# randomwons/RayTracingStudy

Measured on AMD Instinct MI355X. Metric: Mrays/s (primary+shadow) at 1920x1080, 64 spp, 100000 spheres, higher is better.
Workload: dtype f32; 1 GPU; c3: 64 spp Monte-Carlo accumulate, ~100k spheres (headline); width=1920, height=1080, spp=64, n_spheres=100000, octree_depth=7, octree_nodes=37384, prim_refs=153448, leaf_capacity=12, parallelism=single, frames_in_flight=1, rays_per_frame=184963628, primary_per_frame=132710400

## Files before the change

### include/rt.h

```cpp
#ifndef RT_AMD_RT_H
#define RT_AMD_RT_H

#include <stddef.h>
#include <stdint.h>

#ifdef __cplusplus
extern "C" {
#endif

#define RT_ABI_VERSION 4

typedef struct rt_renderer rt_renderer;

enum {
    RT_OK = 0,
    RT_E_INVALID = -1,
    RT_E_HIP = -2,
    RT_E_NOMEM = -3,
    RT_E_NOSCENE = -4,
    RT_E_STATE = -5
};

enum {
    RT_MODE_COMPAT = 0,
    RT_MODE_SCENE = 1
};

enum {
    RT_FLAG_JITTER = 1u << 0,
    RT_FLAG_NO_JITTER = 1u << 1,
    RT_FLAG_RADIANCE = 1u << 2,
    RT_FLAG_NO_SHADOWS = 1u << 3,
    RT_FLAG_HOST_BUILD = 1u << 4,
    RT_FLAG_PROGRESSIVE = 1u << 5,
    RT_FLAG_COMPAT_FMA = 1u << 6,
    RT_FLAG_PAD_FILL_SHIFT = 8,
    RT_FLAG_TEST_HOOKS = 1u << 10,
    RT_FLAG_TEST_POISON = 1u << 11,
    RT_FLAG_NO_OCCLUDERS = 1u << 12,
    RT_FLAG_NO_BINS = 1u << 13,
    RT_FLAG_VARIANT_SHIFT = 16,
    RT_FLAG_OPT_SHIFT = 20,
    RT_FLAG_CELL_TABLE_SHIFT = 28
};

typedef struct rt_config {
    uint32_t width;
    uint32_t height;
    uint32_t spp;
    uint32_t seed;
    int32_t device;
    uint32_t mode;
    uint32_t flags;
    float light_dir[3];
    float ambient;
} rt_config;

typedef struct rt_octree_params {
    float min[3];
    float max[3];
    float resolution;
    uint32_t max_depth;
    uint32_t leaf_capacity;
// ... 58 lines not shown
    RT_BINS_ON = 0,
    RT_BINS_OFF_FLAG = 1,
    RT_BINS_OFF_KERNEL = 2,
    RT_BINS_OFF_CAMERA = 3,
    RT_BINS_OFF_CAPACITY = 4,
    RT_BINS_OFF_WIDE = 5,
    RT_BINS_OFF_DENSE = 6,
    RT_BINS_NO_FRAME = 7
};
typedef struct rt_bin_info {
    uint32_t enabled;
    uint32_t reason;
    uint32_t bin_size;
    uint32_t bins;
    uint32_t entries;
    uint32_t capacity;
    uint32_t non_empty_bins;
    uint32_t longest;
    uint32_t overflowed_bins;
    uint32_t wide;
    float bin_build_ms;
} rt_bin_info;
int rt_get_bin_info(rt_renderer* r, rt_bin_info* info);
int rt_export_bins(rt_renderer* r, uint32_t* headers_out, uint32_t* indices_out, uint32_t* wide_out);
int rt_export_bin_tiles(rt_renderer* r, uint32_t* tw, uint32_t* th, uint32_t* tiles_per_bin,
                        uint64_t* words_out);
int rt_generate_spheres(uint32_t n, uint32_t seed, float* spheres_out, uint32_t* albedo_out);

int rt_save_spheres(const char* path, const float* spheres, const uint32_t* albedo, uint32_t n);
int rt_load_spheres(const char* path, float* spheres_out, uint32_t* albedo_out,
                    uint32_t capacity, uint32_t* n_out);

int rt_render(rt_renderer* r, void* dev_rgba8, void* stream, rt_stats* stats);
int rt_bind_graphics_resource(rt_renderer* r, void* hip_graphics_resource);
typedef struct rt_display_ops {
    int (*map)(void* user, void* stream, void** dev_ptr, size_t* bytes);
    int (*unmap)(void* user, void* stream);
} rt_display_ops;
int rt_bind_display(rt_renderer* r, const rt_display_ops* ops, void* user);
int rt_render_tiles(rt_renderer* r, const uint32_t* tile_ids, uint32_t n_tiles,
                    uint32_t tile_size, void* dev_packed_rgba8, void* stream, rt_stats* stats);
#define RT_TILE_SKIP 0xFFFFFFFFu
int rt_unpack_tiles(rt_renderer* r, const void* dev_packed_rgba8, const uint32_t* tile_ids,
                    uint32_t n_tiles, uint32_t tile_size, void* dev_rgba8, void* stream);
int rt_reset_accumulation(rt_renderer* r);
int rt_synchronize(rt_renderer* r);
// ... 99 lines not shown
```

### raytracingstudy_amd/_lib.py

```python
from __future__ import annotations

import ctypes
import os
import threading

_HERE = os.path.dirname(os.path.abspath(__file__))
LIB_PATH = os.environ.get("RT_AMD_LIB") or os.path.join(_HERE, "librt_amd.so")

RT_OK = 0
RT_E_INVALID = -1
RT_E_HIP = -2
RT_E_NOMEM = -3
RT_E_NOSCENE = -4
RT_E_STATE = -5

RT_MODE_COMPAT = 0
RT_MODE_SCENE = 1

RT_FLAG_JITTER = 1 << 0
RT_FLAG_NO_JITTER = 1 << 1
RT_FLAG_RADIANCE = 1 << 2
RT_FLAG_NO_SHADOWS = 1 << 3
RT_FLAG_HOST_BUILD = 1 << 4
RT_FLAG_PROGRESSIVE = 1 << 5
RT_FLAG_COMPAT_FMA = 1 << 6
RT_BUILDER_DEVICE = 0
RT_BUILDER_HOST = 1
RT_TILE_SKIP = 0xFFFFFFFF
RT_FLAG_PAD_FILL_SHIFT = 8
RT_FLAG_TEST_HOOKS = 1 << 10
RT_FLAG_TEST_POISON = 1 << 11
RT_FLAG_NO_OCCLUDERS = 1 << 12
RT_FLAG_NO_BINS = 1 << 13
RT_FLAG_VARIANT_SHIFT = 16
RT_FLAG_OPT_SHIFT = 20
RT_FLAG_CELL_TABLE_SHIFT = 28
RT_CELL_TABLE_OFF = 15
VARIANT_REMOVED = 2
VARIANT_BLOCK = 7
VARIANT_WAVEQ = 13
VARIANT_WAVEQ_LOW = 4
RT_TRANSPORT_AUTO = 0
RT_TRANSPORT_RCCL = 1
RT_TRANSPORT_PEER = 2
RT_MAX_DEVICES = 16
RT_NO_HIT = 0xFFFFFFFF
RT_QUERY_NEAREST = 0
RT_QUERY_ANY = 1
RT_MULTIHIT_MAX = 16
RT_OVERLAP_MAX = 16
RT_OVERLAP_MORE = 0x80000000
RT_OVERLAP_SKIP_SELF = 1
RT_CLOSEST_MAX = 16
RT_CLOSEST_SKIP_SELF = 1
RT_SWEEP_ENTRY_ONLY = 1
RT_SWEEP_SKIP_SELF = 2
# ... 159 lines not shown
_P = ctypes.c_void_p
_u32 = ctypes.c_uint32
_int = ctypes.c_int
_fp = ctypes.POINTER(ctypes.c_float)
SIGNATURES = {
    "rt_abi_version": (_int, []),
    "rt_device_count": (_int, []),
    "rt_config_default": (None, [ctypes.POINTER(RtConfig)]),
    "rt_octree_params_default": (None, [ctypes.POINTER(RtOctreeParams)]),
    "rt_create": (_int, [ctypes.POINTER(RtConfig), ctypes.POINTER(_P)]),
    "rt_destroy": (_int, [_P]),
    "rt_set_pose": (_int, [_P, _fp]),
    "rt_set_intrinsic": (_int, [_P, _fp]),
    "rt_get_camera": (_int, [_P, _fp, _fp]),
    "rt_resize": (_int, [_P, _u32, _u32]),
    "rt_resize_intrinsic": (None, [_u32, _u32, _fp]),
    "rt_set_scene": (_int, [_P, _P, _P, _u32, ctypes.POINTER(RtOctreeParams)]),
    "rt_set_scene_device": (_int, [_P, _P, _P, _u32, ctypes.POINTER(RtOctreeParams), _P]),
    "rt_set_octree": (_int, [_P, _fp, _fp, ctypes.c_float]),
    "rt_get_scene_info": (_int, [_P, ctypes.POINTER(RtSceneInfo)]),
    "rt_export_octree": (_int, [_P, _P, _P, _P]),
    "rt_export_occluders": (_int, [_P, _P, _P, _P, _P]),
    "rt_get_bin_info": (_int, [_P, ctypes.POINTER(RtBinInfo)]),
    "rt_export_bins": (_int, [_P, _P, _P, _P]),
    "rt_export_bin_tiles": (_int, [_P, _P, _P, _P, _P]),
    "rt_save_spheres": (_int, [ctypes.c_char_p, _P, _P, _u32]),
    "rt_load_spheres": (_int, [ctypes.c_char_p, _P, _P, _u32, ctypes.POINTER(_u32)]),
    "rt_generate_spheres": (_int, [_u32, _u32, _P, _P]),
    "rt_render": (_int, [_P, _P, _P, ctypes.POINTER(RtStats)]),
    "rt_bind_graphics_resource": (_int, [_P, _P]),
    "rt_bind_display": (_int, [_P, ctypes.POINTER(RtDisplayOps), _P]),
    "rt_render_tiles": (_int, [_P, _P, _u32, _u32, _P, _P, ctypes.POINTER(RtStats)]),
    "rt_unpack_tiles": (_int, [_P, _P, _P, _u32, _u32, _P, _P]),
    "rt_trace_rays": (_int, [_P, _P, _u32, _u32, _P, _P, ctypes.POINTER(RtStats)]),
    "rt_pick": (_int, [_P, ctypes.c_float, ctypes.c_float, ctypes.POINTER(RtHit), _fp]),
    "rt_trace_rays_multi": (_int, [_P, _P, _u32, _u32, _P, _P, _P, ctypes.POINTER(RtStats)]),
    "rt_pick_multi": (_int, [_P, ctypes.c_float, ctypes.c_float, _u32, ctypes.POINTER(RtHit),
                             ctypes.POINTER(_u32)]),
    "rt_query_overlaps": (_int, [_P, _P, _u32, _u32, _u32, _P, _P, _P, ctypes.POINTER(RtStats)]),
    "rt_overlaps_at": (_int, [_P, _fp, ctypes.c_float, _u32, ctypes.POINTER(_u32), ctypes.POINTER(_u32)]),
    "rt_query_closest": (_int, [_P, _P, _u32, _u32, _u32, _P, _P, _P, ctypes.POINTER(RtStats)]),
    "rt_closest_at": (_int, [_P, _fp, ctypes.c_float, _u32, ctypes.POINTER(RtNear), ctypes.POINTER(_u32)]),
    "rt_sweep_spheres": (_int, [_P, _P, _P, ctypes.c_float, _u32, _u32, _P, _P, ctypes.POINTER(RtStats)]),
    "rt_sweep_at": (_int, [_P, _fp, _fp, ctypes.c_float, ctypes.c_float, _u32, ctypes.POINTER(RtHit), _fp]),
    "rt_pick_thick": (_int, [_P, ctypes.c_float, ctypes.c_float, ctypes.c_float, ctypes.POINTER(RtHit), _fp]),
    "rt_render_gbuffer": (_int, [_P, ctypes.POINTER(RtGBuffer), _P, ctypes.POINTER(RtStats)]),
# ... 70 lines not shown
```

### raytracingstudy_amd/csrc/rt_capi.cpp

```cpp
#include <mutex>

#include "rt_host.h"

using namespace rtamd;

namespace rtamd {

thread_local std::string g_last_error;

int fail(rt_renderer* r, int code, const std::string& msg) {
    g_last_error = msg;
    if (r) r->err = msg;
    return code;
}

int hip_fail(rt_renderer* r, hipError_t e, const char* what) {
    std::string m = std::string(what) + ": " + hipGetErrorString(e);
    return fail(r, RT_E_HIP, m);
}

int set_device(rt_renderer* r) {
    RT_HIP(r, hipSetDevice(r->device));
    return RT_OK;
}
// ... 362 lines not shown
    if ((st = set_device(r))) return st;
    RT_HIP(r, hipStreamSynchronize(r->stream));
    if (r->pending) RT_HIP(r, hipEventSynchronize(r->done));
    occ_collect_time(r);
    return queue_report(r);
}

int rt_readback(rt_renderer* r, uint8_t* host_rgba8, float* host_rgba32f) {
    if (const int st = rt_synchronize(r)) return st;
    const size_t px = (size_t)r->W * r->H;
    if (host_rgba8) RT_HIP(r, hipMemcpy(host_rgba8, r->fb.p, px * 4, hipMemcpyDeviceToHost));
    if (host_rgba32f) {
        if (!(r->cfg.flags & RT_FLAG_RADIANCE))
            return fail(r, RT_E_STATE, "rt_readback: radiance buffer needs RT_FLAG_RADIANCE");
        RT_HIP(r, hipMemcpy(host_rgba32f, r->rad.p, px * 16, hipMemcpyDeviceToHost));
    }
    return RT_OK;
}

void* rt_framebuffer(rt_renderer* r) { return r ? r->fb.p : nullptr; }

void* rt_stream(rt_renderer* r) { return r ? static_cast<void*>(own_stream(r)) : nullptr; }

const char* rt_last_error(const rt_renderer* r) {
    if (r) return r->err.c_str();
    return g_last_error.c_str();
}

}
```

### raytracingstudy_amd/csrc/rt_frame.cpp

```cpp
#include "rt_frame_math.h"
#include "rt_host.h"

using namespace rtamd;

namespace rtamd {

void fill_frame_args(rt_renderer* r, FrameArgs& a) {
    memset(&a, 0, sizeof(a));
    fill_camera(r, a.cam);
    a.sc = r->sc;
    a.W = r->W;
    a.H = r->H;
    a.spp = r->cfg.spp ? r->cfg.spp : 1;
    a.seedmix = mix32(r->cfg.seed ^ 0x9E3779B9u);
    bool jitter = a.spp > 1;
    if (r->cfg.flags & RT_FLAG_JITTER) jitter = true;
    if (r->cfg.flags & RT_FLAG_NO_JITTER) jitter = false;
    a.jitter = jitter ? 1u : 0u;
    a.shadows = (r->cfg.flags & RT_FLAG_NO_SHADOWS) ? 0u : 1u;
    a.contract = (r->cfg.flags & RT_FLAG_COMPAT_FMA) ? 1u : 0u;
    const float* ld = r->cfg.light_dir;
    const float ll = sqrtf(ld[0] * ld[0] + ld[1] * ld[1] + ld[2] * ld[2]);
    a.L[0] = -(ld[0] / ll);
    a.L[1] = -(ld[1] / ll);
    a.L[2] = -(ld[2] / ll);
    a.ambient = r->cfg.ambient;
    a.inv_spp = 1.0f / static_cast<float>(a.spp);
    if ((r->cfg.flags & RT_FLAG_PROGRESSIVE) && r->cfg.mode == RT_MODE_SCENE) {
        if (uint64_t(r->frames_accum + 1) * a.spp >= (1ull << 31)) r->frames_accum = 0;
        a.accum = r->accum.p;
        a.s_base = r->frames_accum * a.spp;
        a.accum_in = r->frames_accum ? 1u : 0u;
        a.inv_spp = 1.0f / static_cast<float>((r->frames_accum + 1) * a.spp);
    }
    a.counters = r->counters.p;
    a.sc.opt = (r->cfg.flags >> RT_FLAG_OPT_SHIFT) & 0xFFu;
    a.wq_claim_delay = r->test_claim_delay;
    a.qerr = r->qerr_dev;
    if (++r->frame_seq == 0) r->frame_seq = 1;
    a.frame_id = r->frame_seq;
    const uint32_t v = (r->cfg.flags >> RT_FLAG_VARIANT_SHIFT) & 0xFu;
    a.variant = v ? v : default_variant(a.spp);
}

int check_tiles(rt_renderer* r, const uint32_t* ids, uint32_t n_tiles, uint32_t ts,
                bool allow_skip) {
    if (ts == 0 || ts % 64 != 0 || ts > 4096)
        return fail(r, RT_E_INVALID, "tile_size must be a multiple of 64 in [64, 4096]");
    const uint32_t tx = (r->W + ts - 1) / ts, ty = (r->H + ts - 1) / ts;
    for (uint32_t i = 0; i < n_tiles; ++i)
        if (ids[i] >= tx * ty && !(allow_skip && ids[i] == RT_TILE_SKIP))
            return fail(r, RT_E_INVALID, "tile id out of range");
    return RT_OK;
}

constexpr size_t kTileListSlots = 16;

int tile_list(rt_renderer* r, const uint32_t* ids, uint32_t n, hipStream_t s, const uint32_t** out) {
    rt_renderer::TileList* hit = nullptr;
// ... 232 lines not shown
    return RT_OK;
}
int block_stats_end(rt_renderer* r, const FrameArgs& a, hipStream_t st) {
    if (!a.bstats) return RT_OK;
    unsigned long long h[2 * kBlockStats];
    RT_HIP(r, hipStreamSynchronize(st));
    RT_HIP(r, hipMemcpy(h, g_bstats, sizeof(h), hipMemcpyDeviceToHost));
    if (FILE* f = fopen(getenv("RT_BLOCK_STATS_FILE"), "a")) {
        fprintf(f, "{\"W\": %u, \"H\": %u, \"spp\": %u, \"counts\": [", a.W, a.H, a.spp);
        for (uint32_t i = 0; i < 2 * kBlockStats; ++i) fprintf(f, "%s%llu", i ? ", " : "", h[i]);
        fprintf(f, "]}\n");
        fclose(f);
    }
    return RT_OK;
}
#else
inline int block_stats_begin(rt_renderer*, FrameArgs&, hipStream_t) { return RT_OK; }
inline int block_stats_end(rt_renderer*, const FrameArgs&, hipStream_t) { return RT_OK; }
#endif

int launch_frame(rt_renderer* r, FrameArgs& a, const FramePlan* plan, hipStream_t st) {
    int ost;
    if ((ost = timeline_begin(r, a, st)) || (ost = block_stats_begin(r, a, st))) return ost;
    hipError_t e = plan ? launch_scene(a, *plan, st) : launch_compat(a, st);
    counters_after_launch(r, a, e == hipSuccess);
    if (e != hipSuccess) return hip_fail(r, e, "kernel launch");
    if ((ost = block_stats_end(r, a, st)) || (ost = mark_queued(r, st))) return ost;
    if ((ost = timeline_end(r, a, st))) return ost;
    if (a.accum) ++r->frames_accum;
    return RT_OK;
}

int frame_stats(rt_renderer* r, const FrameArgs& a, hipStream_t st, rt_stats* stats) {
    RT_HIP(r, hipEventRecord(r->ev1, st));
    RT_HIP(r, hipEventSynchronize(r->ev1));
    occ_collect_time(r);
    unsigned long long lines[kStatLineWords], c[4];
    RT_HIP(r, hipMemcpy(lines, a.counters + kStatLineBase, sizeof(lines), hipMemcpyDeviceToHost));
    sum_stat_lines(lines, c);
    float ms = 0.f;
    RT_HIP(r, hipEventElapsedTime(&ms, r->ev0, r->ev1));
    memset(stats, 0, sizeof(*stats));
    const uint64_t px = a.tiles ? 0 : (uint64_t)a.W * a.H;
    stats->primary_rays = r->cfg.mode == RT_MODE_SCENE ? c[0] : px;
    stats->shadow_rays = c[1];
    stats->nodes_visited = c[2];
    stats->prims_tested = c[3];
// ... 118 lines not shown
```

### raytracingstudy_amd/csrc/rt_host.h

```cpp
#pragma once
#include <hip/hip_runtime.h>
#include <math.h>
#include <stdio.h>
#include <string.h>

#include <algorithm>
#include <chrono>
#include <string>
#include <vector>

#include "../../include/rt.h"
#include "octree_gpu.h"
#include "rt_bins_math.h"
#include "rt_closest_math.h"
#include "rt_overlap_math.h"
#include "rt_params.h"
#include "rt_sweep_math.h"
#include "scene_build.h"

struct ncclComm;

namespace rtamd {

hipError_t launch_scene(const FrameArgs& a, const FramePlan& plan, hipStream_t st);
bool variant_available(uint32_t v);
hipError_t launch_compat(const FrameArgs& a, hipStream_t st);
hipError_t launch_unpack(const uint32_t* packed, const uint32_t* tiles, uint32_t n_tiles,
                         uint32_t ts, uint32_t tiles_x, uint32_t W, uint32_t H, uint32_t* img,
                         hipStream_t st);
hipError_t launch_cam_screen(const float4* prim_sp, uint32_t n, const float o[3], float4* out,
                             hipStream_t st);
hipError_t launch_shd_screen(const float4* prim_sp, uint32_t n, const float e[6], double delta,
                             float2* out8, uint32_t* rr_max, hipStream_t st);
hipError_t launch_albedo_refs(const uint32_t* prim_idx, const uint32_t* albedo, uint32_t n,
                              uint32_t n_spheres, uint32_t* out, hipStream_t st);
hipError_t launch_cam8_screen(const float4* prim_sp, uint32_t n, const float o[3], const float B[9],
                              uint32_t ok, float2* out, hipStream_t st);
hipError_t launch_query(const FrameArgs& a, const void* rays, void* hits, uint32_t n, bool any,
                        unsigned long long* counters, hipStream_t st);
hipError_t launch_multihit(const FrameArgs& a, const void* rays, void* hits, void* counts, uint32_t n,
                           uint32_t k, unsigned long long* counters, hipStream_t st);
hipError_t launch_overlap(const FrameArgs& a, const void* probes, void* indices, void* counts,
                          uint32_t n, uint32_t k, bool skip_self, float slack_m,
                          unsigned long long* counters, hipStream_t st);
hipError_t launch_closest(const FrameArgs& a, const void* probes, void* near, void* counts, uint32_t n,
                          uint32_t k, bool skip_self, float slack_m, unsigned long long* counters,
                          hipStream_t st);
// ... 203 lines not shown
    uint64_t accum_sig = 0;
    DevBuf<unsigned long long> counters;
    size_t ctr_stride = 0;
    uint32_t ctr_set = 0;
    size_t ctr_zero[2] = {0, 0};
    DevBuf<uint32_t> sb_order;
    uint32_t sb_nx = 0, sb_ny = 0;
    struct TileList {
        std::vector<uint32_t> host;
        DevBuf<uint32_t> dev;
        uint64_t used = 0;
    };
    std::vector<TileList> tile_lists;
    uint64_t tile_clock = 0;
    rt_display_ops disp{};
    void* disp_user = nullptr;
    bool gl_disp = false;
    uint32_t n_spheres = 0;
    std::vector<float> spheres;
    bool host_copy = false;
    uint32_t prim_slots = 0;
    bool leaf_packed = false;
    uint32_t test_claim_delay = 0;
    bool sort_rounds = true, lds_stage = true, leaf_pack = false, sb_hilbert = false;
    rt_octree_params oct;
    bool has_scene = false;
    GpuOctreeBuilder gpu_build;
    CellTable cell_table;
    DevBuf<uint2> d_nodes;
    DevBuf<float4> d_prim_sp;
    DevBuf<uint32_t> d_prim_idx;
    DevBuf<float4> d_spheres;
    DevBuf<uint32_t> d_albedo;
    SceneArgs sc{};
    uint64_t scene_gen = 0;
    DerivedRecords<float4> prim_cam;
    DerivedRecords<float2> prim_cam8;
    DerivedRecords<float2> prim_shd8;
    DevBuf<uint32_t> d_shd_rr;
    uint32_t shd_rr_bits = 0;
    float shd_rr = 0.0f;
    DerivedRecords<uint32_t> prim_al;
    OccluderLists occ;
    uint32_t occ_cap = kOccCap;
    double occ_mean_max = kOccMeanMax;
    hipEvent_t occ_e0 = nullptr, occ_e1 = nullptr;
// ... 68 lines not shown
```

### raytracingstudy_amd/csrc/rt_kernels.hip

```cpp
#include <hip/hip_runtime.h>

#include <algorithm>
#include <mutex>
#include <vector>

#include "rt_params.h"
#include "rt_shade.h"
#include "rt_sorted.h"

namespace rtamd {

__device__ __forceinline__ unsigned long long wave_sum(unsigned long long v) {
#pragma unroll
    for (int off = 32; off > 0; off >>= 1) v += __shfl_xor(v, off, 64);
    return v;
}

__device__ __forceinline__ void flush_counters(const FrameArgs& a, uint32_t prim, uint32_t shadow,
                                               uint32_t nodes, uint32_t prims) {
    const unsigned long long s0 = prim;
    const unsigned long long s1 = shadow;
    const unsigned long long s2 = wave_sum(nodes);
    const unsigned long long s3 = wave_sum(prims);
    if ((threadIdx.x & 63u) == 0) {
// ... 118 lines not shown
                    const uint32_t vc = min(8u, nbx - sx * 8u);
                    const uint32_t r2 = r1 - sx * vr * 8u;
                    sx0 = (sx * 8u + r2 % vc) * 8u;
                    sy0 = (sy * 8u + r2 / vc) * 8u;
                }
                if (kTiles) {
                    const uint32_t tile = a.tiles[k];
                    const uint32_t ts = a.tile_size;
                    tox = (tile % a.tiles_x) * ts;
                    toy = (tile / a.tiles_x) * ts;
                    obase = k * ts * ts - toy * ts - tox;
                }
            }
            for (uint32_t cur = w0; cur < w0 + chunk; ++cur) {
                const uint32_t b = cur >> 6, w = cur & 63u;
                const uint32_t wx = sx0 + (b & 7u) * 8u + (w & 7u);
                const uint32_t wy = sy0 + (b >> 3) * 8u + (w >> 3);
                if (wx >= gw || wy >= gh) continue;
                const uint32_t olx = wx * tw, oly = wy * th;
                const uint32_t ox = olx + tox, oy = oly + toy;
#ifdef RT_TIMELINE
                const unsigned long long tu0 = wall_clock64();
#endif
                if (kSort)
                    shade_pixel_sorted<C>(a, wl, stk, ox, oy, obase, n_primary, n_shadow, n_nodes,
                                          n_prims, bs);
                else
                    shade_wave_tile<C>(a, acc, stk, ox, oy, obase, n_primary, n_shadow, n_nodes,
                                       n_prims, bs, lbs, binc);
#ifdef RT_TIMELINE
                const uint32_t sbt = k * sb_grid + (wy >> 6) * nsx + (wx >> 6);
                const unsigned long long uid = (unsigned long long)sbt * 4096u +
                                               (((wy >> 3) & 7u) * 8u + ((wx >> 3) & 7u)) * 64u +
                                               (wy & 7u) * 8u + (wx & 7u);
                if (a.timeline && (threadIdx.x & 63u) == 0 && uid < (1ull << 22)) {
                    const unsigned hw = __builtin_amdgcn_s_getreg((31 << 11) | 4);
                    const unsigned xcc = __builtin_amdgcn_s_getreg((3 << 11) | 20);
                    a.timeline[4ull * 65536 + 3 * uid] = tu0;
                    a.timeline[4ull * 65536 + 3 * uid + 1] = wall_clock64();
                    a.timeline[4ull * 65536 + 3 * uid + 2] =
                        ((unsigned long long)hw << 32) | (xcc << 16) | (blockIdx.x * 4u + wave);
                }
#endif
            }
        }
    } else {
// ... 129 lines not shown
    const size_t lds = C::waveq ? p.lds_bytes : block_tile_lds(p.lds_bytes, p.spw, a.sc.opt);
    const Occupancy o = occupancy(reinterpret_cast<const void*>(kernel), lds);
    uint32_t grid;
    if constexpr (C::waveq) {
        const WaveQueueLaunch s =
            size_wave_queue(p.grid.units(), o.resident, o.cus, C::min_waves, p.ticket, p.ticket_forced);
        a.wq_chunk = s.ticket;
        grid = s.grid;
    } else {
        const BlockTileLaunch s =
            size_block_tiles(a.W, a.H, a.tiles ? a.n_tiles : 0u, a.tile_size, p.grid.tw, p.grid.th,
                             o.resident, (a.sc.opt >> kOptBtsShift) & 7u);
        a.bts = s.side;
        grid = s.grid;
    }
    hipLaunchKernelGGL(kernel, dim3(grid), dim3(kBlockThreads), lds, st, a);
}

template <uint32_t kT>
static bool launch_flags(uint32_t flags, const FrameArgs& a, const FramePlan& p, hipStream_t st) {
    switch (flags) {
#define RT_INSTANCE(f) \
    case (f): launch_instance<Frame<(f) | kT>>(a, p, st); return true;
#define RT_INSTANCE_OCC(f) RT_INSTANCE(f) RT_INSTANCE((f) | kFOcc)
#define RT_INSTANCE_OCC_BIN(f) RT_INSTANCE_OCC(f) RT_INSTANCE_OCC((f) | kFBin)
        RT_INSTANCE(kFStats)
        RT_INSTANCE(kFStats | kFProg)
        RT_INSTANCE(kFStats | kFWaveQ)
        RT_INSTANCE(kFStats | kFWaveQ | kFProg)
        RT_INSTANCE(kFStats | kFWaveQ | kFSorted)
        RT_INSTANCE(kFStats | kFWaveQ | kFSorted | kFProg)
        RT_INSTANCE_OCC(0u)
        RT_INSTANCE_OCC(kFProg)
        RT_INSTANCE_OCC_BIN(kFWaveQ)
        RT_INSTANCE_OCC_BIN(kFWaveQ | kFProg)
        RT_INSTANCE_OCC_BIN(kFWaveQ | kFSorted)
        RT_INSTANCE_OCC_BIN(kFWaveQ | kFSorted | kFProg)
#undef RT_INSTANCE_OCC_BIN
#undef RT_INSTANCE_OCC
#undef RT_INSTANCE
    }
    return false;
}

bool variant_available(uint32_t v) {
    return pick_scene_instance(v, 1, false, false, false, false, false, 0, 1).valid;
}

hipError_t launch_scene(const FrameArgs& a_in, const FramePlan& p, hipStream_t st) {
    FrameArgs a = a_in;
    const SceneInstance inst =
        p.inst.with(a.sc.prim_occ && a.sc.occ_sp && a.shadows, a.bin_hdr && a.bin_ent && a.bin_info);
    a.spw = p.spw, a.g = p.g, a.ppw = p.ppw, a.rounds = p.rounds;
    a.tw = p.grid.tw, a.th = p.grid.th;
    a.wq_chunk = p.ticket;
    const bool known = inst.valid && (a.tiles ? launch_flags<kFTiles>(inst.flags(), a, p, st)
                                              : launch_flags<0u>(inst.flags(), a, p, st));
    return known ? hipGetLastError() : hipErrorInvalidDeviceFunction;
}

}
```

### raytracingstudy_amd/csrc/rt_sched.h

```cpp
#pragma once
#include <stddef.h>
#include <stdint.h>

#ifdef __HIPCC__
#define RT_HD __host__ __device__
#else
#define RT_HD
#endif

namespace rtamd {

constexpr int kBlockThreads = 256;
constexpr uint32_t kTileSide = 16;

constexpr uint32_t kOptBtsShift = 1;
constexpr uint32_t kOptNoWgCap = 1u << 7;
constexpr uint32_t kOptChunkShift = 4;
constexpr uint32_t kOptChunkMax = 4;

constexpr uint32_t kVariantLaneUnified = 7;
constexpr uint32_t kVariantLaneUnified2NoStats = 10;
constexpr uint32_t kVariantWaveQ = 13;
constexpr uint32_t kVariantWaveQLow = 4;
RT_HD inline uint32_t default_variant(uint32_t spp) { return spp >= 8u ? kVariantWaveQ : kVariantWaveQLow; }

constexpr uint32_t kLeafBuf = 32;
constexpr size_t kLeafBufBytes = (kBlockThreads / 64u) * kLeafBuf * 16u;

constexpr uint32_t kSortMaxRounds = 4;
constexpr uint32_t kSortMax = 64u * kSortMaxRounds;
constexpr uint32_t kSortCellBits = 3;
constexpr uint32_t kSortCells = 1u << (2u * kSortCellBits);
constexpr uint32_t kSortWaveBytes = kSortMax * 8u + 3u * kSortMax + kSortCells * 4u;
static_assert(kSortWaveBytes % 16u == 0u, "per-wave regions stay float4-aligned");

RT_HD inline uint32_t stack_levels(uint32_t tab_k, uint32_t stack_depth, bool no_stack = false) {
    if (no_stack && tab_k) return 0u;
    const uint32_t sb = tab_k ? tab_k - 1u : 0u;
    return stack_depth > 1u + sb ? stack_depth - 1u - sb : 1u;
}

// ... 34 lines not shown
        wave_tile_shape(spp, spw, g, ppw, tw, th);
        gw = n_tiles ? tile_size / tw : (W + tw - 1) / tw;
        gh = n_tiles ? tile_size / th : (H + th - 1) / th;
        nbx = (gw + 7u) / 8u, nby = (gh + 7u) / 8u;
        nsx = (nbx + 7u) / 8u, nsy = (nby + 7u) / 8u;
        grids = n_tiles ? n_tiles : 1u;
    }
    RT_HD uint64_t units() const { return static_cast<uint64_t>(grids) * gw * gh; }
    RT_HD uint32_t blocks() const { return grids * nbx * nby; }
    RT_HD uint32_t superblocks() const { return grids * nsx * nsy; }
    RT_HD uint32_t slot_shift() const { return wave_queue_slot_shift(superblocks(), blocks()); }
    RT_HD uint32_t slot_stride() const { return (slot_shift() == 12u ? superblocks() : blocks()) + 2u; }
};


enum FrameFlag : uint32_t {
    kFTiles = 1u << 0,
    kFStats = 1u << 1,
    kFProg = 1u << 2,
    kFWaveQ = 1u << 3,
    kFSorted = 1u << 4,
    kFOcc = 1u << 5,
    kFBin = 1u << 6,
};

template <uint32_t kF>
struct Frame {
    static constexpr bool tiles = kF & kFTiles, stats = kF & kFStats, prog = kF & kFProg,
                          waveq = kF & kFWaveQ, sorted = kF & kFSorted, occ = kF & kFOcc,
                          bin = kF & kFBin;
    static constexpr int min_waves = waveq ? (stats ? 7 : 8) : 1;
    static constexpr bool cam8 = waveq && !sorted;
    static_assert(!sorted || waveq, "sorted rounds: a wave-queue frame");
    static_assert(!occ || !stats, "stats frames walk: their counters are the oracle's");
    static_assert(!bin || (!stats && waveq), "bins: plain frames of the wave queue");
};

struct SceneInstance {
    bool valid;
    bool waveq, stats, prog, sorted, occ, bin;
    RT_HD uint32_t flags() const {
        return (stats ? kFStats : 0u) | (prog ? kFProg : 0u) | (waveq ? kFWaveQ : 0u) |
               (sorted ? kFSorted : 0u) | (occ ? kFOcc : 0u) | (bin ? kFBin : 0u);
    }
    RT_HD uint32_t min_waves() const { return waveq ? (stats ? 7u : 8u) : 1u; }
    RT_HD bool w8() const { return waveq && !stats; }
    RT_HD SceneInstance with(bool have_occ, bool have_bins) const {
        SceneInstance s = *this;
        s.occ = !stats && have_occ;
        s.bin = !stats && waveq && have_bins;
        return s;
    }
};

RT_HD inline SceneInstance pick_scene_instance(uint32_t variant, uint32_t spp, bool progressive,
                                               bool count_work, bool sort_on, bool have_occ,
                                               bool have_bins, uint32_t tab_k, uint32_t stack_depth) {
    if (!variant) variant = default_variant(spp);
    SceneInstance s = {true, false, count_work, progressive, false, false, false};
    const uint32_t rounds = (spp + 63u) / 64u;
    s.sorted = sort_on && spp >= 64u && rounds >= 2u && rounds <= kSortMaxRounds &&
               FrameLds(true, tab_k, stack_depth).bytes * 8u <= 160u * 1024u &&
               (progressive || variant == kVariantWaveQ);
    if (s.sorted)
        s.waveq = true;
    else if (progressive)
        s.waveq = spp >= 8u;
    else if (variant == kVariantWaveQ || variant == kVariantWaveQLow)
        s.waveq = true;
    else if (variant == kVariantLaneUnified)
        s.stats = true;
    else if (variant != kVariantLaneUnified2NoStats)
        s.valid = false;
    return s.with(have_occ, have_bins);
}


struct FramePlan {
    SceneInstance inst;
    WaveGrid grid;
    uint32_t spw, g, ppw, rounds;
    uint32_t slot_shift, slot_stride;
    uint32_t lds_bytes;
    uint32_t ticket;
    bool ticket_forced;
};

RT_HD inline FramePlan plan_scene_frame(uint32_t variant, uint32_t spp, bool progressive, bool count_work,
                                        bool sort_on, uint32_t tab_k, uint32_t stack_depth, uint32_t W,
                                        uint32_t H, uint32_t n_tiles, uint32_t tile_size, uint32_t opt) {
    FramePlan p = {pick_scene_instance(variant, spp, progressive, count_work, sort_on, false, false, tab_k,
                                       stack_depth),
                   WaveGrid(W, H, spp, n_tiles, tile_size)};
    uint32_t tw, th;
    wave_tile_shape(spp, p.spw, p.g, p.ppw, tw, th);
    p.rounds = (spp + p.spw - 1) / p.spw;
    p.slot_shift = p.grid.slot_shift();
    p.slot_stride = p.grid.slot_stride();
    p.lds_bytes = FrameLds(p.inst.sorted, tab_k, stack_depth).bytes;
    const uint32_t ck = (opt >> kOptChunkShift) & 7u;
    p.ticket = ck ? 1u << (ck - 1u) : 4u / (p.rounds < 1u ? 1u : p.rounds > 4u ? 4u : p.rounds);
    p.ticket_forced = ck != 0u;
    return p;
}


struct WaveQueueLaunch {
    uint32_t grid, ticket;
};
struct BlockTileLaunch {
    uint32_t grid, side;
};

RT_HD inline WaveQueueLaunch size_wave_queue(uint64_t units, uint32_t resident, uint32_t cus, uint32_t per_simd,
                                        uint32_t ticket, bool ticket_forced) {
    const uint64_t want = (units + kBlockThreads / 64 - 1) / (kBlockThreads / 64);
    const uint64_t cap = per_simd ? static_cast<uint64_t>(cus) * per_simd : resident;
    uint64_t grid = resident < cap ? resident : cap;
    if (want < grid) grid = want;
    if (grid < 1u) grid = 1u;
    WaveQueueLaunch s = {static_cast<uint32_t>(grid), ticket};
    if (!ticket_forced) {
        const uint64_t per_wave = units / (grid * (kBlockThreads / 64));
        const uint32_t most = per_wave >= 64 ? 4u : per_wave >= 16 ? 2u : 1u;
        if (most < s.ticket) s.ticket = most;
    }
// ... 29 lines not shown
```

### raytracingstudy_amd/csrc/rt_shade.h

```cpp
#pragma once
#include <hip/hip_runtime.h>

#include "rt_params.h"
#include "rt_walk.h"
#include "rt_bins.h"

namespace rtamd {

__device__ __forceinline__ float sat(float x) { return x > 0.0f ? (x < 1.0f ? x : 1.0f) : 0.0f; }

__device__ __forceinline__ uint32_t mix32(uint32_t x) {
    x ^= x >> 16;
    x *= 0x7feb352du;
    x ^= x >> 15;
    x *= 0x846ca68bu;
    x ^= x >> 16;
    return x;
}

__device__ __forceinline__ float u01(uint32_t x) {
    return static_cast<float>(x >> 8) * (1.0f / 16777216.0f);
}

__device__ __forceinline__ void get_ray(const CamArgs& c, float u, float v, float& wx, float& wy,
// ... 165 lines not shown
                c.b = A.z + c.b;
            }
            acc[threadIdx.x] = make_float4(c.r, c.g, c.b, 0.0f);
        }
    }
    KernArgs* ko = kernargs();
    if (leader) {
        const float4 A = acc[threadIdx.x];
        if (kProg) ko->accum[(size_t)y * ko->W + x] = A;
        const float isp = ko->inv_spp;
        const PixelOut p{A.x * isp, A.y * isp, A.z * isp};
        const uint32_t rgba = pack_rgba8(p);
        if (kTiles) {
            ko->out8[obase + y * ko->tile_size + x] = rgba;
        } else {
            ko->out8[(size_t)y * ko->W + x] = rgba;
            if (ko->out32) ko->out32[(size_t)y * ko->W + x] = make_float4(p.r, p.g, p.b, 1.0f);
        }
    } else if (kTiles && sub == 0 && pix < ko->ppw) {
        ko->out8[obase + y * ko->tile_size + x] = 0u;
    }
}

}
```

### raytracingstudy_amd/renderer.py

```python
from __future__ import annotations

import ctypes
from typing import Optional, Sequence

import numpy as np

from . import _lib
from ._lib import (RT_FLAG_HOST_BUILD, RT_FLAG_JITTER, RT_FLAG_NO_JITTER, RT_FLAG_NO_SHADOWS,
                   RT_FLAG_PROGRESSIVE, RT_FLAG_RADIANCE,
                   RT_MODE_COMPAT, RT_MODE_SCENE, RtConfig, RtOctreeParams, RtSceneInfo,
                   RtStats, check)

__all__ = ["KernelRenderer", "resize_intrinsic", "generate_spheres", "device_count",
           "save_spheres", "load_spheres"]

_MODES = {"compat": RT_MODE_COMPAT, "scene": RT_MODE_SCENE}
_QUERY_KINDS = {"nearest": _lib.RT_QUERY_NEAREST, "any": _lib.RT_QUERY_ANY}


def _fptr(a: np.ndarray):
    return a.ctypes.data_as(ctypes.POINTER(ctypes.c_float))


def _vptr(a: Optional[np.ndarray]):
# ... 62 lines not shown
    return sp[:n.value], al[:n.value]


def _octree_params(root_min, root_max, resolution, max_depth, leaf_capacity) -> RtOctreeParams:
    p = RtOctreeParams()
    for i in range(3):
        p.min[i] = float(root_min[i])
        p.max[i] = float(root_max[i])
    p.resolution = float(resolution)
    p.max_depth = int(max_depth)
    p.leaf_capacity = int(leaf_capacity)
    return p


class KernelRenderer:

    def __init__(self, width: int, height: int, *, mode: str = "compat", spp: int = 1,
                 seed: int = 0x2545F491, device: int = -1, jitter: Optional[bool] = None,
                 shadows: bool = True, radiance: bool = False,
                 light_dir: Sequence[float] = (1.0, 1.0, -1.0), ambient: float = 0.1,
                 variant: int = 0, opt_off: int = 0, host_build: bool = False,
                 progressive: bool = False, cell_table: Optional[int] = None,
                 compat_fma: bool = False, pad_fill: int = 0, occluders: bool = True,
                 bins: bool = True,
                 devices: Optional[Sequence[int]] = None, transport: str = "auto"):
        lib = _lib.load()
        cfg = RtConfig()
        lib.rt_config_default(ctypes.byref(cfg))
        cfg.width, cfg.height = int(width), int(height)
        cfg.spp = int(spp)
        cfg.seed = int(seed) & 0xFFFFFFFF
        cfg.device = int(device)
        cfg.mode = _MODES[mode]
        flags = 0
        if jitter is True:
            flags |= RT_FLAG_JITTER
        elif jitter is False:
            flags |= RT_FLAG_NO_JITTER
        if not shadows:
            flags |= RT_FLAG_NO_SHADOWS
        if radiance:
            flags |= RT_FLAG_RADIANCE
        if host_build:
            flags |= RT_FLAG_HOST_BUILD
        if progressive:
            flags |= RT_FLAG_PROGRESSIVE
        if compat_fma:
            flags |= _lib.RT_FLAG_COMPAT_FMA
        if not occluders:
            flags |= _lib.RT_FLAG_NO_OCCLUDERS
        if not bins:
            flags |= _lib.RT_FLAG_NO_BINS
        if not 0 <= int(pad_fill) <= 2:
            raise ValueError("pad_fill must be 0, 1 or 2")
        flags |= int(pad_fill) << _lib.RT_FLAG_PAD_FILL_SHIFT
        flags |= (int(variant) & 0xF) << _lib.RT_FLAG_VARIANT_SHIFT
        flags |= (int(opt_off) & 0xFF) << _lib.RT_FLAG_OPT_SHIFT
        if cell_table is not None:
            ct = _lib.RT_CELL_TABLE_OFF if int(cell_table) == 0 else int(cell_table)
            if not 1 <= ct <= 15:
                raise ValueError("cell_table must be None, 0 (off) or a depth 1..7")
            flags |= ct << _lib.RT_FLAG_CELL_TABLE_SHIFT
        cfg.flags = flags | _lib.test_flags
        for i in range(3):
            cfg.light_dir[i] = float(light_dir[i])
        cfg.ambient = float(ambient)
        self._lib = lib
        self.config = cfg
        self.mode = mode
        self.radiance = radiance
        h = ctypes.c_void_p()
        if devices is None:
            check(lib.rt_create(ctypes.byref(cfg), ctypes.byref(h)))
        else:
            tr = {"auto": _lib.RT_TRANSPORT_AUTO, "rccl": _lib.RT_TRANSPORT_RCCL,
# ... 82 lines not shown
        nodes = np.zeros((max(info["n_nodes"], 1), 2), np.uint32)
        m = info["n_prim_refs"]
        sp = np.zeros((max(m, 1), 4), np.float32)
        idx = np.zeros(max(m, 1), np.uint32)
        check(self._lib.rt_export_octree(self._h, _vptr(nodes), _vptr(sp), _vptr(idx)), self._h)
        return nodes[:info["n_nodes"]], sp[:m], idx[:m]

    def export_occluders(self):
        info = self.scene_info()
        n, m, e = info["n_spheres"], info["n_prim_refs"], info["occluder_entries"]
        off = np.zeros(max(n, 1), np.uint32)
        cnt = np.zeros(max(n, 1), np.uint32)
        idx = np.zeros(max(e, 1), np.uint32)
        refs = np.zeros((max(m, 1), 2), np.uint32)
        check(self._lib.rt_export_occluders(self._h, _vptr(off), _vptr(cnt), _vptr(idx), _vptr(refs)),
              self._h)
        return off[:n], cnt[:n], idx[:e], refs[:m]

    def bin_info(self) -> dict:
        info = _lib.RtBinInfo()
        check(self._lib.rt_get_bin_info(self._h, ctypes.byref(info)), self._h)
        return info.as_dict()

    def export_bins(self):
        bi = self.bin_info()
        hdr = np.zeros((max(bi["bins"], 1), 2), np.uint32)
        idx = np.zeros(max(bi["entries"], 1), np.uint32)
        wide = np.zeros(max(bi["wide"], 1), np.uint32)
        check(self._lib.rt_export_bins(self._h, _vptr(hdr), _vptr(idx), _vptr(wide)), self._h)
        return hdr[:bi["bins"]], idx[:bi["entries"]], wide[:bi["wide"]]

    def export_bin_tiles(self):
        bi = self.bin_info()
        tw, th, tpb = ctypes.c_uint32(), ctypes.c_uint32(), ctypes.c_uint32()
        check(self._lib.rt_export_bin_tiles(self._h, ctypes.byref(tw), ctypes.byref(th), ctypes.byref(tpb),
                                            None), self._h)
        words = np.zeros((max(bi["bins"], 1), tpb.value), np.uint64)
        check(self._lib.rt_export_bin_tiles(self._h, None, None, None, _vptr(words)), self._h)
        return (tw.value, th.value), words[:bi["bins"]]

    def scene_info(self) -> dict:
        info = RtSceneInfo()
        check(self._lib.rt_get_scene_info(self._h, ctypes.byref(info)), self._h)
        return info.as_dict()

    def multi_info(self) -> dict:
# ... 255 lines not shown
```

Baseline: 150,100 Mrays/s.

## Shade horizontal pixel pairs per wave to share bin traversal

Adds a pair path in which one wave shades two adjacent pixels together. It walks the union of both pixels' bin bitmasks once, loading each entry a single time and testing it against both rays, then resolves both pixels' occluder lists in one loop. The path runs only for binned, occluder-enabled plain frames with one pixel per wave and one round, and it falls back to the single-pixel path for walk bins. The cost is more registers and divergence, since lanes idle when one pixel's list is longer. A flag to disable it and an accessor reporting the launched instance are also added.

```diff
diff --git a/include/rt.h b/include/rt.h
--- a/include/rt.h
+++ b/include/rt.h
@@ -39,6 +39,7 @@
     RT_FLAG_TEST_POISON = 1u << 11,
     RT_FLAG_NO_OCCLUDERS = 1u << 12,
     RT_FLAG_NO_BINS = 1u << 13,
+    RT_FLAG_NO_PAIRS = 1u << 14,
     RT_FLAG_VARIANT_SHIFT = 16,
     RT_FLAG_OPT_SHIFT = 20,
     RT_FLAG_CELL_TABLE_SHIFT = 28
@@ -143,6 +144,7 @@
     float bin_build_ms;
 } rt_bin_info;
 int rt_get_bin_info(rt_renderer* r, rt_bin_info* info);
+uint32_t rt_last_instance(const rt_renderer* r);
 int rt_export_bins(rt_renderer* r, uint32_t* headers_out, uint32_t* indices_out, uint32_t* wide_out);
 int rt_export_bin_tiles(rt_renderer* r, uint32_t* tw, uint32_t* th, uint32_t* tiles_per_bin,
                         uint64_t* words_out);
diff --git a/raytracingstudy_amd/_lib.py b/raytracingstudy_amd/_lib.py
--- a/raytracingstudy_amd/_lib.py
+++ b/raytracingstudy_amd/_lib.py
@@ -32,6 +32,7 @@
 RT_FLAG_TEST_POISON = 1 << 11
 RT_FLAG_NO_OCCLUDERS = 1 << 12
 RT_FLAG_NO_BINS = 1 << 13
+RT_FLAG_NO_PAIRS = 1 << 14
 RT_FLAG_VARIANT_SHIFT = 16
 RT_FLAG_OPT_SHIFT = 20
 RT_FLAG_CELL_TABLE_SHIFT = 28
@@ -237,6 +238,7 @@
     "rt_export_octree": (_int, [_P, _P, _P, _P]),
     "rt_export_occluders": (_int, [_P, _P, _P, _P, _P]),
     "rt_get_bin_info": (_int, [_P, ctypes.POINTER(RtBinInfo)]),
+    "rt_last_instance": (_u32, [_P]),
     "rt_export_bins": (_int, [_P, _P, _P, _P]),
     "rt_export_bin_tiles": (_int, [_P, _P, _P, _P, _P]),
     "rt_save_spheres": (_int, [ctypes.c_char_p, _P, _P, _u32]),
diff --git a/raytracingstudy_amd/csrc/rt_capi.cpp b/raytracingstudy_amd/csrc/rt_capi.cpp
--- a/raytracingstudy_amd/csrc/rt_capi.cpp
+++ b/raytracingstudy_amd/csrc/rt_capi.cpp
@@ -408,6 +408,8 @@
 
 void* rt_stream(rt_renderer* r) { return r ? static_cast<void*>(own_stream(r)) : nullptr; }
 
+uint32_t rt_last_instance(const rt_renderer* r) { return r ? r->last_instance : 0u; }
+
 const char* rt_last_error(const rt_renderer* r) {
     if (r) return r->err.c_str();
     return g_last_error.c_str();
diff --git a/raytracingstudy_amd/csrc/rt_frame.cpp b/raytracingstudy_amd/csrc/rt_frame.cpp
--- a/raytracingstudy_amd/csrc/rt_frame.cpp
+++ b/raytracingstudy_amd/csrc/rt_frame.cpp
@@ -34,7 +34,7 @@
         a.inv_spp = 1.0f / static_cast<float>((r->frames_accum + 1) * a.spp);
     }
     a.counters = r->counters.p;
-    a.sc.opt = (r->cfg.flags >> RT_FLAG_OPT_SHIFT) & 0xFFu;
+    a.sc.opt = ((r->cfg.flags >> RT_FLAG_OPT_SHIFT) & 0xFFu) | ((r->cfg.flags & RT_FLAG_NO_PAIRS) ? kOptNoPairs : 0u);
     a.wq_claim_delay = r->test_claim_delay;
     a.qerr = r->qerr_dev;
     if (++r->frame_seq == 0) r->frame_seq = 1;
@@ -313,7 +313,7 @@
 int launch_frame(rt_renderer* r, FrameArgs& a, const FramePlan* plan, hipStream_t st) {
     int ost;
     if ((ost = timeline_begin(r, a, st)) || (ost = block_stats_begin(r, a, st))) return ost;
-    hipError_t e = plan ? launch_scene(a, *plan, st) : launch_compat(a, st);
+    hipError_t e = plan ? launch_scene(a, *plan, st, &r->last_instance) : launch_compat(a, st);
     counters_after_launch(r, a, e == hipSuccess);
     if (e != hipSuccess) return hip_fail(r, e, "kernel launch");
     if ((ost = block_stats_end(r, a, st)) || (ost = mark_queued(r, st))) return ost;
diff --git a/raytracingstudy_amd/csrc/rt_host.h b/raytracingstudy_amd/csrc/rt_host.h
--- a/raytracingstudy_amd/csrc/rt_host.h
+++ b/raytracingstudy_amd/csrc/rt_host.h
@@ -22,7 +22,7 @@
 
 namespace rtamd {
 
-hipError_t launch_scene(const FrameArgs& a, const FramePlan& plan, hipStream_t st);
+hipError_t launch_scene(const FrameArgs& a, const FramePlan& plan, hipStream_t st, uint32_t* instance);
 bool variant_available(uint32_t v);
 hipError_t launch_compat(const FrameArgs& a, hipStream_t st);
 hipError_t launch_unpack(const uint32_t* packed, const uint32_t* tiles, uint32_t n_tiles,
@@ -272,6 +272,7 @@
     uint32_t prim_slots = 0;
     bool leaf_packed = false;
     uint32_t test_claim_delay = 0;
+    uint32_t last_instance = 0;
     bool sort_rounds = true, lds_stage = true, leaf_pack = false, sb_hilbert = false;
     rt_octree_params oct;
     bool has_scene = false;
diff --git a/raytracingstudy_amd/csrc/rt_kernels.hip b/raytracingstudy_amd/csrc/rt_kernels.hip
--- a/raytracingstudy_amd/csrc/rt_kernels.hip
+++ b/raytracingstudy_amd/csrc/rt_kernels.hip
@@ -164,6 +164,13 @@
 #ifdef RT_TIMELINE
                 const unsigned long long tu0 = wall_clock64();
 #endif
+                if constexpr (C::pair) {
+                    if (pair_starts(cur, w0, chunk) &&
+                        shade_pixel_pair<C>(ox, oy, n_primary, n_shadow, binc)) {
+                        ++cur;
+                        continue;
+                    }
+                }
                 if (kSort)
                     shade_pixel_sorted<C>(a, wl, stk, ox, oy, obase, n_primary, n_shadow, n_nodes,
                                           n_prims, bs);
@@ -339,6 +346,8 @@
     switch (flags) {
 #define RT_INSTANCE(f) \
     case (f): launch_instance<Frame<(f) | kT>>(a, p, st); return true;
+#define RT_INSTANCE_FRAME(f) \
+    case (f): if constexpr (kT == 0u) { launch_instance<Frame<(f)>>(a, p, st); return true; } else return false;
 #define RT_INSTANCE_OCC(f) RT_INSTANCE(f) RT_INSTANCE((f) | kFOcc)
 #define RT_INSTANCE_OCC_BIN(f) RT_INSTANCE_OCC(f) RT_INSTANCE_OCC((f) | kFBin)
         RT_INSTANCE(kFStats)
@@ -353,6 +362,8 @@
         RT_INSTANCE_OCC_BIN(kFWaveQ | kFProg)
         RT_INSTANCE_OCC_BIN(kFWaveQ | kFSorted)
         RT_INSTANCE_OCC_BIN(kFWaveQ | kFSorted | kFProg)
+        RT_INSTANCE_FRAME(kFWaveQ | kFOcc | kFBin | kFPair)
+#undef RT_INSTANCE_FRAME
 #undef RT_INSTANCE_OCC_BIN
 #undef RT_INSTANCE_OCC
 #undef RT_INSTANCE
@@ -364,13 +375,15 @@
     return pick_scene_instance(v, 1, false, false, false, false, false, 0, 1).valid;
 }
 
-hipError_t launch_scene(const FrameArgs& a_in, const FramePlan& p, hipStream_t st) {
+hipError_t launch_scene(const FrameArgs& a_in, const FramePlan& p, hipStream_t st, uint32_t* instance) {
     FrameArgs a = a_in;
-    const SceneInstance inst =
+    SceneInstance inst =
         p.inst.with(a.sc.prim_occ && a.sc.occ_sp && a.shadows, a.bin_hdr && a.bin_ent && a.bin_info);
+    if (a.tiles) inst.pair = false;
     a.spw = p.spw, a.g = p.g, a.ppw = p.ppw, a.rounds = p.rounds;
     a.tw = p.grid.tw, a.th = p.grid.th;
     a.wq_chunk = p.ticket;
+    *instance = inst.flags() | (a.tiles ? kFTiles : 0u);
     const bool known = inst.valid && (a.tiles ? launch_flags<kFTiles>(inst.flags(), a, p, st)
                                               : launch_flags<0u>(inst.flags(), a, p, st));
     return known ? hipGetLastError() : hipErrorInvalidDeviceFunction;
diff --git a/raytracingstudy_amd/csrc/rt_sched.h b/raytracingstudy_amd/csrc/rt_sched.h
--- a/raytracingstudy_amd/csrc/rt_sched.h
+++ b/raytracingstudy_amd/csrc/rt_sched.h
@@ -17,6 +17,7 @@
 constexpr uint32_t kOptNoWgCap = 1u << 7;
 constexpr uint32_t kOptChunkShift = 4;
 constexpr uint32_t kOptChunkMax = 4;
+constexpr uint32_t kOptNoPairs = 1u << 8;
 
 constexpr uint32_t kVariantLaneUnified = 7;
 constexpr uint32_t kVariantLaneUnified2NoStats = 10;
@@ -97,26 +98,30 @@
     kFSorted = 1u << 4,
     kFOcc = 1u << 5,
     kFBin = 1u << 6,
+    kFPair = 1u << 7,
 };
 
 template <uint32_t kF>
 struct Frame {
     static constexpr bool tiles = kF & kFTiles, stats = kF & kFStats, prog = kF & kFProg,
                           waveq = kF & kFWaveQ, sorted = kF & kFSorted, occ = kF & kFOcc,
-                          bin = kF & kFBin;
+                          bin = kF & kFBin, pair = kF & kFPair;
     static constexpr int min_waves = waveq ? (stats ? 7 : 8) : 1;
     static constexpr bool cam8 = waveq && !sorted;
     static_assert(!sorted || waveq, "sorted rounds: a wave-queue frame");
     static_assert(!occ || !stats, "stats frames walk: their counters are the oracle's");
     static_assert(!bin || (!stats && waveq), "bins: plain frames of the wave queue");
+    static_assert(!pair || (bin && occ && !sorted && !prog && !tiles),
+                  "pairs: binned plain frames with occluder lists, not packed tiles");
 };
 
 struct SceneInstance {
     bool valid;
     bool waveq, stats, prog, sorted, occ, bin;
+    bool pair_shape, pair;
     RT_HD uint32_t flags() const {
         return (stats ? kFStats : 0u) | (prog ? kFProg : 0u) | (waveq ? kFWaveQ : 0u) |
-               (sorted ? kFSorted : 0u) | (occ ? kFOcc : 0u) | (bin ? kFBin : 0u);
+               (sorted ? kFSorted : 0u) | (occ ? kFOcc : 0u) | (bin ? kFBin : 0u) | (pair ? kFPair : 0u);
     }
     RT_HD uint32_t min_waves() const { return waveq ? (stats ? 7u : 8u) : 1u; }
     RT_HD bool w8() const { return waveq && !stats; }
@@ -124,6 +129,7 @@
         SceneInstance s = *this;
         s.occ = !stats && have_occ;
         s.bin = !stats && waveq && have_bins;
+        s.pair = pair_shape && s.bin && s.occ && !sorted && !prog;
         return s;
     }
 };
@@ -132,7 +138,7 @@
                                                bool count_work, bool sort_on, bool have_occ,
                                                bool have_bins, uint32_t tab_k, uint32_t stack_depth) {
     if (!variant) variant = default_variant(spp);
-    SceneInstance s = {true, false, count_work, progressive, false, false, false};
+    SceneInstance s = {true, false, count_work, progressive, false, false, false, false, false};
     const uint32_t rounds = (spp + 63u) / 64u;
     s.sorted = sort_on && spp >= 64u && rounds >= 2u && rounds <= kSortMaxRounds &&
                FrameLds(true, tab_k, stack_depth).bytes * 8u <= 160u * 1024u &&
@@ -170,6 +176,7 @@
     uint32_t tw, th;
     wave_tile_shape(spp, p.spw, p.g, p.ppw, tw, th);
     p.rounds = (spp + p.spw - 1) / p.spw;
+    p.inst.pair_shape = p.ppw == 1u && p.rounds == 1u && !(opt & kOptNoPairs);
     p.slot_shift = p.grid.slot_shift();
     p.slot_stride = p.grid.slot_stride();
     p.lds_bytes = FrameLds(p.inst.sorted, tab_k, stack_depth).bytes;
@@ -177,6 +184,10 @@
     p.ticket = ck ? 1u << (ck - 1u) : 4u / (p.rounds < 1u ? 1u : p.rounds > 4u ? 4u : p.rounds);
     p.ticket_forced = ck != 0u;
     return p;
+}
+
+RT_HD inline bool pair_starts(uint32_t cur, uint32_t w0, uint32_t chunk) {
+    return (cur & 1u) == 0u && cur + 1u < w0 + chunk;
 }
 
 
diff --git a/raytracingstudy_amd/csrc/rt_shade.h b/raytracingstudy_amd/csrc/rt_shade.h
--- a/raytracingstudy_amd/csrc/rt_shade.h
+++ b/raytracingstudy_amd/csrc/rt_shade.h
@@ -211,4 +211,181 @@
     }
 }
 
-}
+
+typedef uint32_t pair_u32x4 __attribute__((ext_vector_type(4), aligned(8)));
+
+struct PairRay {
+    float d0, d1, d2;
+};
+
+__device__ __forceinline__ PairRay pair_ray(KernArgs* ka, uint32_t x, uint32_t y, uint32_t hp, uint32_t s) {
+    float u = static_cast<float>(x), v = static_cast<float>(y);
+    if (ka->jitter) {
+        u = u + u01(mix32(hp ^ (s << 1)));
+        v = v + u01(mix32(hp ^ ((s << 1) | 1u)));
+    }
+    CamArgs cam;
+    for (int i = 0; i < 9; ++i) cam.K[i] = ka->cam.K[i], cam.R[i] = ka->cam.R[i];
+    PairRay r;
+    get_ray(cam, u, v, r.d0, r.d1, r.d2);
+    return r;
+}
+
+struct PairShade {
+    float lam, o0, o1, o2;
+    bool want;
+};
+__device__ __forceinline__ PairShade pair_shade(KernArgs* kb, float4 sp, float r0, float r1, float r2,
+                                                const PairRay& d, float t, bool hit) {
+    const float p0 = r0 + t * d.d0;
+    const float p1 = r1 + t * d.d1;
+    const float p2 = r2 + t * d.d2;
+    const float ir = 1.0f / sp.w;
+    const float n0 = (p0 - sp.x) * ir;
+    const float n1 = (p1 - sp.y) * ir;
+    const float n2 = (p2 - sp.z) * ir;
+    const float ndl = n0 * kb->L[0] + n1 * kb->L[1] + n2 * kb->L[2];
+    PairShade s;
+    s.lam = hit && ndl > 0.0f ? ndl : 0.0f;
+    s.want = hit && ndl > 0.0f && kb->shadows;
+    s.o0 = p0 + n0 * kShadowEps;
+    s.o1 = p1 + n1 * kShadowEps;
+    s.o2 = p2 + n2 * kShadowEps;
+    return s;
+}
+
+__device__ __forceinline__ PixelOut pair_color(float amb, bool hit, float lam, uint32_t al, const PairRay& d) {
+    PixelOut c{200.0f / 255.0f, sat(d.d1), sat(d.d2)};
+    if (hit) {
+        const float f = amb + (1.0f - amb) * lam;
+        c.r = static_cast<float>(al & 0xFFu) * (1.0f / 255.0f) * f;
+        c.g = static_cast<float>((al >> 8) & 0xFFu) * (1.0f / 255.0f) * f;
+        c.b = static_cast<float>((al >> 16) & 0xFFu) * (1.0f / 255.0f) * f;
+    }
+    return c;
+}
+
+template <class C>
+__device__ __forceinline__ bool shade_pixel_pair(uint32_t ox, uint32_t oy, uint32_t& n_primary,
+                                                 uint32_t& n_shadow, uint32_t binc) {
+    static_assert(C::pair && !C::tiles, "a frame instance with the pair path");
+    KernArgs* ka = kernargs();
+    const uint32_t W = ka->W;
+    if (bin_consts_flag(binc)) return false;
+    const uint32_t b = (oy >> kBinShift) * ka->bin_nbx + (ox >> kBinShift);
+    const bin_u32x2 h = *reinterpret_cast<__attribute__((address_space(4))) const bin_u32x2*>(
+        reinterpret_cast<uintptr_t>(ka->bin_hdr + b));
+    const size_t wi = (static_cast<size_t>(b) << (2u * kBinShift)) + bin_tile_index_log2(ox, oy, 0u, 0u);
+    const pair_u32x4 w = *reinterpret_cast<__attribute__((address_space(4))) const pair_u32x4*>(
+        reinterpret_cast<uintptr_t>(ka->bin_hdr + ka->bin_nb + wi));
+    if (h.y == kBinWalk) return false;
+    const bool b_on = ox + 1u < W;
+    unsigned long long wa = h.y ? (static_cast<unsigned long long>(w.y) << 32) | w.x : 0ull;
+    unsigned long long wb = h.y && b_on ? (static_cast<unsigned long long>(w.w) << 32) | w.z : 0ull;
+
+    uint32_t tid = threadIdx.x;
+    asm volatile("" : "+v"(tid));
+    const uint32_t lane = tid & 63u;
+    const bool va = lane < ka->spw, vb = va && b_on;
+    const uint32_t pid = oy * W + ox;
+    const uint32_t seedmix = ka->seedmix;
+    const PairRay da = pair_ray(ka, ox, oy, mix32(seedmix ^ pid), lane);
+    const PairRay db = pair_ray(ka, ox + 1u, oy, mix32(seedmix ^ (pid + 1u)), lane);
+    const float r0 = ka->cam.o[0], r1 = ka->cam.o[1], r2 = ka->cam.o[2];
+
+    BinBest ba{va ? INFINITY : -INFINITY, kNoHit, kNoHit};
+    BinBest bb{vb ? INFINITY : -INFINITY, kNoHit, kNoHit};
+    BinEntries* ent = reinterpret_cast<BinEntries*>(reinterpret_cast<uintptr_t>(ka->bin_ent)) + h.x;
+    while (wa | wb) {
+        const uint32_t k = static_cast<uint32_t>(__builtin_ctzll(wa | wb));
+        const unsigned long long bit = 1ull << k;
+        const bin_u32x8 e = ent[k];
+        const bool in_a = (wa & bit) != 0ull, in_b = (wb & bit) != 0ull;
+        wa &= ~bit;
+        wb &= ~bit;
+        if (in_a && !bin_entry(e, r0, r1, r2, da.d0, da.d1, da.d2, ba)) wa = 0ull;
+        if (in_b && !bin_entry(e, r0, r1, r2, db.d0, db.d1, db.d2, bb)) wb = 0ull;
+    }
+    const uint32_t nw = bin_consts_wide(binc);
+    if (nw) {
+        BinEntries* wide = reinterpret_cast<BinEntries*>(reinterpret_cast<uintptr_t>(ka->bin_wide));
+        bool on_a = true, on_b = b_on;
+        for (uint32_t k = 0; k < nw && (on_a || on_b); ++k) {
+            const bin_u32x8 e = wide[k];
+            if (on_a) on_a = bin_entry(e, r0, r1, r2, da.d0, da.d1, da.d2, ba);
+            if (on_b) on_b = bin_entry(e, r0, r1, r2, db.d0, db.d1, db.d2, bb);
+        }
+    }
+    const bool hit_a = ba.ref != kNoHit, hit_b = bb.ref != kNoHit;
+
+    float lam_a = 0.0f, lam_b = 0.0f;
+    uint32_t al_a = 0, al_b = 0;
+    uint2 occ_a = make_uint2(0u, 0u), occ_b = make_uint2(0u, 0u);
+    PairShade sa{0.0f, 0.0f, 0.0f, 0.0f, false}, sb = sa;
+    if (hit_a || hit_b) {
+        KernArgs* kb = kernargs();
+        const uint32_t ia = hit_a ? ba.ref : bb.ref, ib = hit_b ? bb.ref : ba.ref;
+        const float4 sp_a = kb->sc.prim_sp[ia];
+        const float4 sp_b = kb->sc.prim_sp[ib];
+        al_a = kb->sc.prim_al[ia];
+        al_b = kb->sc.prim_al[ib];
+        occ_a = kb->sc.prim_occ[ia];
+        occ_b = kb->sc.prim_occ[ib];
+        sa = pair_shade(kb, sp_a, r0, r1, r2, da, ba.t, hit_a);
+        sb = pair_shade(kb, sp_b, r0, r1, r2, db, bb.t, hit_b);
+        lam_a = sa.lam, lam_b = sb.lam;
+    }
+    const bool want_a = sa.want, want_b = sb.want;
+    if (__any((want_a && occ_a.y == kOccWalk) || (want_b && occ_b.y == kOccWalk))) return false;
+    if (want_a || want_b) {
+        KernArgs* kl = kernargs();
+        const float l0 = kl->L[0], l1 = kl->L[1], l2 = kl->L[2];
+        const float4* __restrict__ lst = kl->sc.occ_sp;
+        const uint32_t cnt_a = want_a ? occ_a.y : 0u, cnt_b = want_b ? occ_b.y : 0u;
+        bool oc_a = false, oc_b = false;
+        for (uint32_t k = 0;; ++k) {
+            const bool go_a = k < cnt_a && !oc_a, go_b = k < cnt_b && !oc_b;
+            if (!(go_a || go_b)) break;
+            const float4 ca = lst[go_a ? occ_a.x + k : 0u];
+            const float4 cb = lst[go_b ? occ_b.x + k : 0u];
+            float th;
+            const bool xa = isect(sa.o0, sa.o1, sa.o2, l0, l1, l2, ca, 0.0f, INFINITY, th);
+            const bool xb = isect(sb.o0, sb.o1, sb.o2, l0, l1, l2, cb, 0.0f, INFINITY, th);
+            oc_a = go_a ? xa : oc_a;
+            oc_b = go_b ? xb : oc_b;
+        }
+        if (oc_a) lam_a = 0.0f;
+        if (oc_b) lam_b = 0.0f;
+    }
+    n_primary += static_cast<uint32_t>(__popcll(__ballot(va)) + __popcll(__ballot(vb)));
+    n_shadow += static_cast<uint32_t>(__popcll(__ballot(want_a)) + __popcll(__ballot(want_b)));
+
+    const float amb = kernargs()->ambient;
+    PixelOut ca = pair_color(amb, hit_a, lam_a, al_a, da);
+    PixelOut cb = pair_color(amb, hit_b, lam_b, al_b, db);
+    if (!va) ca = PixelOut{0.0f, 0.0f, 0.0f};
+    if (!vb) cb = PixelOut{0.0f, 0.0f, 0.0f};
+#pragma unroll
+    for (uint32_t m = 1; m < 64u; m <<= 1) {
+        const float ar = __shfl_xor(ca.r, static_cast<int>(m), 64), ag = __shfl_xor(ca.g, static_cast<int>(m), 64),
+                    ab = __shfl_xor(ca.b, static_cast<int>(m), 64), br = __shfl_xor(cb.r, static_cast<int>(m), 64),
+                    bg = __shfl_xor(cb.g, static_cast<int>(m), 64), bl = __shfl_xor(cb.b, static_cast<int>(m), 64);
+        ca.r += ar, ca.g += ag, ca.b += ab;
+        cb.r += br, cb.g += bg, cb.b += bl;
+    }
+    KernArgs* ko = kernargs();
+    if (lane < 2u) {
+        const bool second = lane != 0u;
+        const float isp = ko->inv_spp;
+        const PixelOut p{(second ? cb.r : ca.r) * isp, (second ? cb.g : ca.g) * isp, (second ? cb.b : ca.b) * isp};
+        const uint32_t rgba = pack_rgba8(p);
+        if (!second || b_on) {
+            const size_t o = (size_t)oy * ko->W + ox + lane;
+            ko->out8[o] = rgba;
+            if (ko->out32) ko->out32[o] = make_float4(p.r, p.g, p.b, 1.0f);
+        }
+    }
+    return true;
+}
+
+}
diff --git a/raytracingstudy_amd/renderer.py b/raytracingstudy_amd/renderer.py
--- a/raytracingstudy_amd/renderer.py
+++ b/raytracingstudy_amd/renderer.py
@@ -108,7 +108,7 @@
                  variant: int = 0, opt_off: int = 0, host_build: bool = False,
                  progressive: bool = False, cell_table: Optional[int] = None,
                  compat_fma: bool = False, pad_fill: int = 0, occluders: bool = True,
-                 bins: bool = True,
+                 bins: bool = True, pairs: bool = True,
                  devices: Optional[Sequence[int]] = None, transport: str = "auto"):
         lib = _lib.load()
         cfg = RtConfig()
@@ -137,6 +137,8 @@
             flags |= _lib.RT_FLAG_NO_OCCLUDERS
         if not bins:
             flags |= _lib.RT_FLAG_NO_BINS
+        if not pairs:
+            flags |= _lib.RT_FLAG_NO_PAIRS
         if not 0 <= int(pad_fill) <= 2:
             raise ValueError("pad_fill must be 0, 1 or 2")
         flags |= int(pad_fill) << _lib.RT_FLAG_PAD_FILL_SHIFT
@@ -265,6 +267,9 @@
         check(self._lib.rt_get_bin_info(self._h, ctypes.byref(info)), self._h)
         return info.as_dict()
 
+    def last_instance(self) -> int:
+        return int(self._lib.rt_last_instance(self._h))
+
     def export_bins(self):
         bi = self.bin_info()
         hdr = np.zeros((max(bi["bins"], 1), 2), np.uint32)
```

After: 167,200 Mrays/s (median of 6 runs). 11.4% higher.
